# tigert1998/ray-tracing-cuda

Hardware: AMD Instinct MI355X
Metric: Mrays/s (higher is better)
Workload: dtype f32

## Files before the change

### include/rtmi.h

```cpp
#ifndef RTMI_H_
#define RTMI_H_

#include <stddef.h>
#include <stdint.h>

#ifdef __cplusplus
extern "C" {
#endif

#define RTMI_VERSION 3
#define RTMI_TILE 8
#define RTMI_STATE_WORDS 6

typedef enum rtmi_status {
  RTMI_OK = 0,
  RTMI_ERR_INVALID = -1,
  RTMI_ERR_NO_DEVICE = -2,
  RTMI_ERR_HIP = -3,
  RTMI_ERR_CAPACITY = -4,
  RTMI_ERR_DEPTH = -5,
  RTMI_ERR_INTERNAL = -6
} rtmi_status;

#define RTMI_MAX_DEPTH 64
// ... 94 lines not shown

int rtmi_post_process(float *d_image, int64_t n_pixels, int spp, void *stream);
int rtmi_get_workload(int rank, int world_size, int spp);

int rtmi_selftest_arithmetic(unsigned long long mismatches[8]);

typedef struct rtmi_render_opts {
  int32_t size;
  int32_t schedule;
  int32_t blocks_per_cu;
  int32_t threads_per_block;
  int32_t sparse_stride;
  int32_t exclusive;
  int32_t outlier_x10;
  int32_t probe_spp;
  int32_t head_pct[3];
  int32_t plan;
  int32_t wave_priority;
  int32_t lane_stride;
  int32_t promote_after;
  int32_t cost_probe;
  int32_t first_pass;
  int32_t fast_path;
  void *d_scratch;
  size_t scratch_bytes;
} rtmi_render_opts;
size_t rtmi_render_scratch_bytes(const rtmi_frame *f);
int rtmi_render_launch_shape(const rtmi_scene *s, const rtmi_frame *f, const rtmi_render_opts *opts, int32_t out[4]);
int rtmi_render_mode(const rtmi_scene *s, const rtmi_frame *f, const rtmi_render_opts *opts, int32_t out[8]);
#define RTMI_MODE_FIELDS 9
int rtmi_render_mode_ex(const rtmi_scene *s, const rtmi_frame *f, const rtmi_render_opts *opts, int32_t *out, int n);
#define RTMI_FAST_PATH_FACTS 14
int rtmi_fast_path_kernel(const int32_t facts[RTMI_FAST_PATH_FACTS]);
int rtmi_render_ex(const rtmi_scene *s, const rtmi_frame *f, const rtmi_render_opts *opts, void *d_states,
                   float *d_tiles, uint32_t *d_ray_counts, void *stream);

enum {
  RTMI_HIT_NONE = 0,
  RTMI_HIT_SPHERE = 1,
  RTMI_HIT_TRIANGLE = 2,
  RTMI_HIT_PARALLELOGRAM = 3,
  RTMI_HIT_PARALLELEPIPED = 4,
  RTMI_HIT_MESH = 5,
  RTMI_HIT_SKY = 6
};
typedef struct rtmi_hit {
  float t;
  float u, v;
  float normal[3];
  int32_t material;
  int32_t kind;
  int32_t entry;
  int32_t element;
  int32_t reserved[2];
} rtmi_hit;

int rtmi_intersect(const rtmi_scene *s, int64_t n, const float *d_origins, const float *d_dirs,
                   const float *d_t_max, rtmi_hit *d_hits, unsigned long long *d_abandoned, void *stream);

int rtmi_occluded(const rtmi_scene *s, int64_t n, const float *d_origins, const float *d_dirs, const float *d_t_max,
                  uint8_t *d_occluded, unsigned long long *d_counts, void *stream);

#define RTMI_TRACE_WORK_WORDS 256
int rtmi_trace(const rtmi_scene *s, int64_t n, const float *d_origins, const float *d_dirs, int max_depth,
               void *d_states, float *d_radiance, uint32_t *d_ray_counts, unsigned long long *d_work, void *stream);
int rtmi_rng_init_n(uint64_t seed, uint64_t first, int64_t n, void *d_states, void *stream);
// ... 177 lines not shown
```

### ray-tracing-cuda_amd/csrc/capi.hip

```cpp
#include <hip/hip_runtime.h>
#include <dlfcn.h>
#include <rccl/rccl.h>
#include <string.h>

#include <algorithm>
#include <cmath>
#include <cstdlib>
#include <mutex>
#include <string>
#include <type_traits>
#include <unordered_map>

#include "../../include/rtmi.h"
#include "kernels.h"
#include "scene.h"
#include "xorwow.h"

using namespace rtmi;

static thread_local std::string g_err;
static int fail(int code, const std::string &msg) {
  g_err = msg;
  return code;
}
// ... 351 lines not shown
int rtmi_camera_set(rtmi_scene *s, const float f[21], int is_defocus, double lens_radius) {
  if (!s || !f) return fail(RTMI_ERR_INVALID, "null argument");
  CameraDev &c = S(s)->cam;
  c.position = v3(f), c.llc = v3(f + 3), c.horizontal = v3(f + 6), c.vertical = v3(f + 9);
  c.u = v3(f + 12), c.v = v3(f + 15);
  S(s)->cam_w = v3(f + 18);
  c.defocus = is_defocus ? 1 : 0;
  c.lens_radius = (float)lens_radius;
  S(s)->has_camera = true;
  S(s)->committed = false;
  return RTMI_OK;
}
int rtmi_camera_update(rtmi_scene *s, const float f[21], int is_defocus, double lens_radius) {
  if (!s || !f) return fail(RTMI_ERR_INVALID, "null argument");
  if (!all_finite(f, 21)) return fail(RTMI_ERR_INVALID, "non-finite camera float");
  Scene *sc = S(s);
  const bool committed = sc->committed;
  if (int rc = rtmi_camera_set(s, f, is_defocus, lens_radius)) return rc;
  if (committed) {
    sc->dev.cam = sc->cam;
    sc->features = sc->cam.defocus ? sc->features | F_DEFOCUS : sc->features & ~(uint32_t)F_DEFOCUS;
    sc->committed = true;
  }
  return RTMI_OK;
}
int rtmi_camera_get(const rtmi_scene *s, float out[21]) {
  if (!s || !out || !S(s)->has_camera) return fail(RTMI_ERR_INVALID, "scene has no camera");
  const CameraDev &c = S(s)->cam;
  const V3 vs[7] = {c.position, c.llc, c.horizontal, c.vertical, c.u, c.v, S(s)->cam_w};
  for (int i = 0; i < 7; i++) out[i * 3] = vs[i].x, out[i * 3 + 1] = vs[i].y, out[i * 3 + 2] = vs[i].z;
  return RTMI_OK;
}

int rtmi_scene_commit(rtmi_scene *sp) {
  if (!sp) return fail(RTMI_ERR_INVALID, "null scene");
  Scene *s = S(sp);
  if (s->list_counts.size() != 1) return fail(RTMI_ERR_INVALID, "a nested list is still open (rtmi_list_end missing)");
  static_assert(RTMI_MAX_MATERIALS == kMaxMats, "rtmi.h and scene_dev.h disagree on the material limit");
  if (s->mats.size() > (size_t)RTMI_MAX_MATERIALS)
    return fail(RTMI_ERR_CAPACITY, "more than RTMI_MAX_MATERIALS (2^24) materials: a triangle's material field has 24 bits");
  if (rtmi_device_count() <= 0) return fail(RTMI_ERR_NO_DEVICE, "no HIP device: librtmi has no CPU fallback");
  free_device(s);
  std::string err = s->flatten();
  if (!err.empty()) return fail(RTMI_ERR_INVALID, err);
  HIP_TRY(hipGetDevice(&s->device));
  s->tex_recs.clear();
  for (const HostTex &t : s->texs) {
    if (!t.image) continue;
    void *d = nullptr;
    size_t pitch = 0;
    HIP_TRY(hipMallocPitch(&d, &pitch, (size_t)t.w * 4, (size_t)t.h));
    s->dev_allocs.push_back(d);
    HIP_TRY(hipMemcpy2D(d, pitch, t.rgba.data(), (size_t)t.w * 4, (size_t)t.w * 4, (size_t)t.h,
                        hipMemcpyHostToDevice));
    TexRec r{};
    r.rgba = reinterpret_cast<const uint8_t *>(d);
    r.height = t.h, r.width = t.w, r.pitch = (int64_t)pitch;
    s->tex_recs.push_back(r);
  }
  SceneDev d{};
  int rc;
  if ((rc = upload(s, s->runs, &d.runs))) return rc;
  if ((rc = upload(s, s->spheres, &d.spheres))) return rc;
  if ((rc = upload(s, s->tris, &d.tris))) return rc;
  {
    static_assert(sizeof(PairSlab) == sizeof(PairBox) && std::is_trivially_copyable<PairSlab>::value, "PairSlab records travel as PairBox");
// ... 12 lines not shown
  if ((rc = upload(s, s->nodes, &d.nodes))) return rc;
  if ((rc = upload(s, s->qnodes, &d.qnodes))) return rc;
  if ((rc = upload(s, s->leaf_paths, &d.leaf_paths))) return rc;
  if ((rc = upload(s, s->tops, &d.tops))) return rc;
  if ((rc = upload(s, s->faces, &d.faces))) return rc;
  if ((rc = upload(s, s->face_uv, &d.face_uv))) return rc;
#ifdef RTMI_CHECK_MARGINS
  if ((rc = upload(s, s->face_of_orig, &d.face_of_orig))) return rc;
#endif
  if ((rc = upload(s, s->mat_recs, &d.mats))) return rc;
  if ((rc = upload(s, s->tex_recs, &d.texs))) return rc;
  d.n_runs = (int)s->runs.size() - 4;
  d.n_pairs = (int)s->pair_pts.size();
  d.list_mag = s->list_mag;
  d.n_mats = (int)s->mat_recs.size();
  d.n_nodes = (int)s->nodes.size();
  d.n_leaf_paths = (int)s->leaf_paths.size();
  d.sub_reserve = s->sub_depth > 0 ? 3 * s->sub_depth + 3 + kMeshFaceSlack : 0;
  d.det_safe = 1;
  for (const HotTri &t : s->tris) {
    const double a = std::sqrt((double)t.e1[0] * t.e1[0] + (double)t.e1[1] * t.e1[1] + (double)t.e1[2] * t.e1[2]);
    const double b = std::sqrt((double)t.e2[0] * t.e2[0] + (double)t.e2[1] * t.e2[1] + (double)t.e2[2] * t.e2[2]);
    if (!(a * b <= 0x1p120)) d.det_safe = 0;
  }
  d.unsigned_colours = 1;
  for (const MatRec &m : s->mat_recs) {
    const float c[3] = {m.r, m.g, m.b};
    for (float x : c) {
      uint32_t bits;
      memcpy(&bits, &x, sizeof(bits));
      if (bits >> 31) d.unsigned_colours = 0;
    }
  }
  d.cam = s->cam;
  s->dev = d;
  QueryDev q{};
  if ((rc = upload(s, s->q_sphere_entry, &q.sphere_entry))) return rc;
  if ((rc = upload(s, s->q_pair_entry, &q.pair_entry))) return rc;
  if ((rc = upload(s, s->q_bvh_entry, &q.bvh_entry))) return rc;
  if ((rc = upload(s, s->q_face_input, &q.face_input))) return rc;
  q.sky_entry = s->q_sky_entry;
  s->qdev = q;
  {
    std::vector<uint32_t> light_mats;
    std::vector<LightRec> recs;
    std::vector<float> cdf;
    build_light_table(*s, &s->lights, &light_mats);
    light_records(s->lights, &recs, &cdf);
    LightDev l{};
    if ((rc = upload(s, recs, &l.recs))) return rc;
    if ((rc = upload(s, cdf, &l.cdf))) return rc;
    if ((rc = upload(s, light_mats, &l.light_mats))) return rc;
    l.n_lights = (int32_t)s->lights.size(), l.n_mats = (int32_t)s->mat_recs.size();
    std::vector<int32_t> hit_light;
    build_hit_light_map(s->lights, &hit_light, &l.n_entries);
    if ((rc = upload(s, hit_light, &l.hit_light))) return rc;
    s->ldev = l;
  }
  void *c = nullptr;
  HIP_TRY(hipMalloc(&c, RTMI_COUNTER_WORDS * sizeof(unsigned long long) + 2 * render_params_bytes()));
  s->dev_allocs.push_back(c);
  HIP_TRY(hipMemset(c, 0, RTMI_COUNTER_WORDS * sizeof(unsigned long long)));
  s->d_counters = reinterpret_cast<unsigned long long *>(c);
  HIP_TRY(hipDeviceSynchronize());
  s->committed = true;
  return RTMI_OK;
// ... 35 lines not shown
}

int64_t rtmi_debug_list_records(const rtmi_scene *sp, int64_t cap_pairs, uint32_t *tri_pts, uint32_t *hot_tris, float *corners) {
  if (!sp) return fail(RTMI_ERR_INVALID, "null scene");
  Scene tmp;
  if (int rc = flattened(sp, &tmp)) return rc;
  const int64_t n = (int64_t)tmp.pair_pts.size();
  for (int64_t i = 0; i < n && i < cap_pairs; i++) {
    if (tri_pts) memcpy(tri_pts + 24 * i, &tmp.tri_pts[2 * i], 2 * sizeof(TriPts));
    if (hot_tris) memcpy(hot_tris + 32 * i, &tmp.tris[2 * i], 2 * sizeof(HotTri));
    if (corners) memcpy(corners + 12 * i, tmp.pair_pts[i].p0, 12 * sizeof(float));
  }
  return n;
}

int64_t rtmi_debug_pair_slabs(const rtmi_scene *sp, int64_t cap, uint32_t *slabs, uint32_t *boxes, float *list_mag) {
  if (!sp) return fail(RTMI_ERR_INVALID, "null scene");
  Scene tmp;
  if (int rc = flattened(sp, &tmp)) return rc;
  const int64_t n = (int64_t)tmp.pair_slabs.size();
  for (int64_t i = 0; i < n && i < cap; i++) {
    if (slabs) memcpy(slabs + 8 * i, &tmp.pair_slabs[i], sizeof(PairSlab));
    if (boxes) memcpy(boxes + 8 * i, &tmp.pair_boxes[i], sizeof(PairBox));
  }
  if (list_mag) *list_mag = tmp.list_mag;
  return n;
}

int rtmi_debug_slab_reach(const rtmi_scene *sp) {
  if (!sp) return fail(RTMI_ERR_INVALID, "null scene");
  Scene tmp;
  if (int rc = flattened(sp, &tmp)) return rc;
  return slab_reach_covers(tmp.list_mag, tmp.cam) ? 1 : 0;
}

int64_t rtmi_debug_render_lds_bytes(const rtmi_scene *sp, int max_depth, int threads) {
  if (!sp || max_depth < 0 || threads < 64 || threads % 64) return fail(RTMI_ERR_INVALID, "bad arguments");
  Scene tmp;
  if (int rc = flattened(sp, &tmp)) return rc;
  SceneDev d{};
  d.n_pairs = (int)tmp.pair_pts.size(), d.n_mats = (int)tmp.mat_recs.size(), d.n_nodes = (int)tmp.nodes.size();
  d.n_leaf_paths = (int)tmp.leaf_paths.size(), d.n_sph_groups = (int)tmp.sph_groups.size();
  FrameDev fr{};
  fr.max_depth = max_depth;
  return (int64_t)render_lds_bytes(pick_variant(tmp.features), d, fr, threads);
}

int64_t rtmi_frame_work_items(const rtmi_frame *f) {
  FrameDev d;
  if (!make_frame(f, &d)) return fail(RTMI_ERR_INVALID, frame_why("bad frame"));
  return d.items;
}
int64_t rtmi_frame_pixel_of(const rtmi_frame *f, int64_t q) {
  FrameDev d;
  if (!make_frame(f, &d) || q < 0 || q >= d.items) return -1;
  return frame_pixel_of(d, d.rank, q);
}
int rtmi_frame_pixel_map(const rtmi_frame *f, int64_t *out) {
  FrameDev d;
  if (!make_frame(f, &d) || !out) return fail(RTMI_ERR_INVALID, frame_why("bad frame"));
  for (int64_t q = 0; q < d.items; q++) out[q] = frame_pixel_of(d, d.rank, q);
  return RTMI_OK;
}
size_t rtmi_states_bytes(const rtmi_frame *f) {
  FrameDev d;
  if (!make_frame(f, &d)) return 0;
// ... 245 lines not shown
  p->scratch = p->scheduled || p->prio;
  p->first = p->finish = d;
  p->first.k_end = probe_spp;
  if (p->resume) p->finish.k_begin = probe_spp;
  else p->first.spp = probe_spp;
  p->first_fast = fast_mode(ls.fast, ls.lane_stride, p->first_prio, false, false, false);
  p->finish_fast = fast_mode(ls.fast, ls.lane_stride, p->prio, p->chains, p->resume, p->scheduled);
  return RTMI_OK;
}

int rtmi_render_launch_shape(const rtmi_scene *sp, const rtmi_frame *f, const rtmi_render_opts *opts, int32_t out[4]) {
  if (!sp || !out) return fail(RTMI_ERR_INVALID, "null argument");
  RenderPlan p;
  int rc;
  if ((rc = render_prologue(sp, f, opts, &p)) || (rc = plan_render(&p))) return rc;
  out[0] = p.ls.blocks, out[1] = p.ls.threads, out[2] = p.ls.per_cu, out[3] = p.ls.n_cu;
  return RTMI_OK;
}

int rtmi_render_mode(const rtmi_scene *sp, const rtmi_frame *f, const rtmi_render_opts *opts, int32_t out[8]) {
  return rtmi_render_mode_ex(sp, f, opts, out, 8);
}
int rtmi_render_mode_ex(const rtmi_scene *sp, const rtmi_frame *f, const rtmi_render_opts *opts, int32_t *dst, int n) {
  if (!sp || !dst || n < 0) return fail(RTMI_ERR_INVALID, "null argument");
  RenderPlan p;
  int rc;
  if ((rc = render_prologue(sp, f, opts, &p)) || (rc = plan_render(&p))) return rc;
  const int32_t out[RTMI_MODE_FIELDS] = {p.scheduled, p.scheduled ? p.probe_spp : 0, p.resume, p.chains, p.prio ? p.tune.prio_every : 0,
                                         p.ls.lane_stride, p.waves, p.d.local_tiles, p.finish_fast != 0u};
  for (int i = 0; i < n && i < RTMI_MODE_FIELDS; i++) dst[i] = out[i];
  return RTMI_OK;
}

struct Scratch {
  uint32_t *states, *rays, *cost, *order, *meta, *head, *work, *qcost, *qsorted, *qmap, *qmax, *fut, *claims, *prio_tab;
  int32_t *next, *first;
};
static Scratch scratch_regions(void *base, const ScratchLayout &l) {
  const auto at = [base](size_t off) { return reinterpret_cast<uint32_t *>(static_cast<char *>(base) + off); };
  const auto ints = [&at](size_t off) { return reinterpret_cast<int32_t *>(at(off)); };
  return Scratch{at(l.states), at(l.rays), at(l.cost), at(l.order), at(l.meta), at(l.head), at(l.work), at(l.qcost), at(l.qsorted),
                 at(l.qmap), at(l.qmax), at(l.fut), at(l.claims), at(l.prio_tab), ints(l.next), ints(l.first)};
}

struct SchedStep {
  int tiles;
  bool pixel_head;
  uint32_t sparse_cap;
  int waves, outlier_x10;
  const int *head_pct;
  int simds, rounds;
  int spp, probe_spp;
};
static int schedule_step(const Scratch &r, uint32_t *rays, const uint32_t *work, const SchedStep &k, SchedPlan *plan,
                         hipStream_t st) {
  uint32_t *head = k.pixel_head ? r.head : nullptr;
  HIP_TRY(launch_tile_order(rays, k.tiles, r.cost, r.meta, r.order, head, k.sparse_cap, k.waves, k.outlier_x10, k.head_pct, st));
  HIP_TRY(launch_quarter_order(r.order, work, rays, k.tiles, r.qcost, r.qsorted, r.qmax, r.qmap, st));
  plan->tile_order = r.qmap;
  plan->sparse_items = r.meta + 1;
  plan->head_list = head;
  plan->probe_marks = head ? rays : nullptr;
  plan->probe_spp = k.probe_spp;
  plan->tile_cost = r.cost;
  if ((int64_t)k.simds * k.rounds > 0) {
    HIP_TRY(launch_chain_plan(r.order, r.cost, k.tiles, k.simds, k.rounds, k.spp, k.probe_spp, r.first, r.next, r.fut, st));
// ... 903 lines not shown
```

### ray-tracing-cuda_amd/csrc/kernels.h

```cpp
#pragma once
#include <hip/hip_runtime.h>
#include <stdint.h>

#include <vector>

#include "../../include/rtmi.h"
#include "scene_dev.h"

#define RTMI_KERNEL_MAX_DEPTH 64

namespace rtmi {

#include "path_list.h"

int64_t frame_pixel_of(const FrameDev &fr, int rank, int64_t q);

hipError_t launch_rng_init(uint64_t seed, const FrameDev &fr, const uint32_t *d_jump, uint32_t *d_states,
                           hipStream_t stream, int64_t first = -1);

uint32_t pick_variant(uint32_t features);
int render_occupancy(uint32_t variant, const SceneDev &sc, const FrameDev &fr, int threads, bool fast_path = false);
struct RenderTuning {
  int schedule;
  int blocks_per_cu;
  int threads;
  int sparse_stride;
  int exclusive;
  int outlier_x10;
  int head_pct[3];
  int probe_spp;
  int promote;
  int first_pass;
  int cost_probe;
  int lane_stride;
  int plan;
  int prio_every;
  int fast_path;
  int head_classes;
  int first_prio;
  int fetch_batch, fetch_batch_first;
};

enum : uint32_t {
  PIN_NIBBLE_IDS = 1u << 0,
  PIN_LDS_TABLES = 1u << 1,
  PIN_UNSIGNED = 1u << 2,
  PIN_DET_SAFE = 1u << 3,
  PIN_POW2_FRAME = 1u << 4,
  PIN_EVERY_LANE = 1u << 5,
  PIN_PRIORITIES = 1u << 6,
  PIN_CHAINS = 1u << 7,
  PIN_QUEUE = 1u << 8,
};
constexpr uint32_t kFastCommon = PIN_NIBBLE_IDS | PIN_LDS_TABLES | PIN_UNSIGNED | PIN_DET_SAFE | PIN_POW2_FRAME |
                                 PIN_EVERY_LANE | PIN_PRIORITIES;
constexpr uint32_t kFastChains = kFastCommon | PIN_CHAINS;
constexpr uint32_t kFastQueue = kFastCommon | PIN_QUEUE;
constexpr bool defers_unit(uint32_t m) { return (m & kFastCommon) == kFastCommon; }
constexpr bool culls_by_slab(uint32_t m) { return (m & kFastCommon) == kFastCommon; }
constexpr bool folds_by_min(uint32_t m) { return (m & kFastCommon) == kFastCommon; }
#ifndef RTMI_TRIM
#define RTMI_TRIM 7
#endif
constexpr bool trims_votes(uint32_t m) { return (RTMI_TRIM & 1) && (m & kFastCommon) == kFastCommon; }
constexpr bool trims_mul24(uint32_t m) { return (RTMI_TRIM & 2) && (m & kFastCommon) == kFastCommon; }
constexpr bool trims_fold_rgb(uint32_t m) { return (RTMI_TRIM & 4) && (m & kFastCommon) == kFastCommon; }
constexpr int kFoldRgbOff = 512;
constexpr int kFoldRgbBytes = 256;
constexpr int kOrderedTasksWord = 16;
struct FastPathFacts {
  int enabled;
  uint32_t variant;
  int n_mats;
  int mats_in_lds;
  int pairs_in_lds;
  int unsigned_colours;
  int det_safe;
  int width, height;
  int lane_stride;
  int priorities;
  int chains;
  int resumed;
  int tile_cost;
};
uint32_t fast_path_mode(const FastPathFacts &f);
FastPathFacts fast_path_facts(uint32_t variant, const SceneDev &sc, const FrameDev &fr, int threads, int enabled);
bool slab_reach_covers(float list_mag, const CameraDev &cam);
size_t render_lds_bytes(uint32_t variant, const SceneDev &sc, const FrameDev &fr, int threads);
struct SchedPlan {
  const uint32_t *tile_order = nullptr;
  uint32_t *visit_counts = nullptr;
  const uint32_t *sparse_items = nullptr;
  const uint32_t *head_list = nullptr;
  const uint32_t *probe_marks = nullptr;
  int probe_spp = 2;
  uint32_t *prio_tab = nullptr;
  const uint32_t *tile_cost = nullptr;
  const int32_t *chain_next = nullptr;
  const uint32_t *chain_fut = nullptr;
// ... 122 lines not shown
```

### ray-tracing-cuda_amd/csrc/render.hip

```cpp
#include <hip/hip_runtime.h>
#include <stdint.h>

#include "kernels.h"

#include <cfloat>
#include <cmath>
#include <cstdlib>
#include <iterator>
#include <type_traits>
#include "scene_dev.h"
#include "vec.h"
#include "xorwow.h"

namespace rtmi {

#include "frame_math.h"
#include "trace_helpers.h"
#include "path_shared.h"
#include "mesh_search.h"
#include "closest_hit.h"
#include "render_body.h"
#include "launch_cfg.h"

size_t render_params_bytes() { return (sizeof(RenderParams) + 255) & ~(size_t)255; }
// ... 85 lines not shown
bool slab_reach_covers(float list_mag, const CameraDev &cam) {
  const float reach = kOriginReach * list_mag;
  const bool cam_in_reach = fabsf(cam.position.x) <= reach && fabsf(cam.position.y) <= reach && fabsf(cam.position.z) <= reach;
  const bool k_finite = (double)(kOriginReach + 1.0f) * (double)list_mag * 1e30 < (double)FLT_MAX;
  return cam_in_reach && k_finite;
}
FastPathFacts fast_path_facts(uint32_t variant, const SceneDev &sc, const FrameDev &fr, int threads, int enabled) {
  size_t lds = 0;
  const LaunchCfg lc = make_cfg(variant, sc, fr, threads, &lds);
  FastPathFacts f{};
  f.enabled = enabled, f.variant = variant, f.n_mats = sc.n_mats, f.mats_in_lds = lc.lds_mats > 0 && lc.wide_ids == 2;
  f.pairs_in_lds = lc.pairs_off >= 0 && lc.nrm_off >= 0 && lc.list_off >= 0 && slab_reach_covers(sc.list_mag, sc.cam);
  f.unsigned_colours = sc.unsigned_colours, f.det_safe = sc.det_safe, f.width = fr.width, f.height = fr.height;
  return f;
}

size_t render_lds_bytes(uint32_t variant, const SceneDev &sc, const FrameDev &fr, int threads) {
  size_t lds = 0;
  (void)make_cfg(variant, sc, fr, threads, &lds);
  return lds;
}

int render_occupancy(uint32_t variant, const SceneDev &sc, const FrameDev &fr, int threads, bool fast_path) {
  return with_listed<kVariants>(variant, 0, [&](auto v) {
    constexpr uint32_t F = decltype(v)::value;
    size_t lds = 0;
    (void)make_cfg(F, sc, fr, threads, &lds);
    if (threads > RTMI_MAX_THREADS(F)) return 0;
    int nb = 0;
    (void)kernel_occupancy<render_kernel<F>>(threads, lds, &nb);
    if constexpr (F == (uint32_t)F_TRIS) {
      if (fast_path) {
        int nc = 0, nq = 0;
        (void)kernel_occupancy<render_kernel<F, kFastChains>>(threads, lds, &nc);
        (void)kernel_occupancy<render_kernel<F, kFastQueue>>(threads, lds, &nq);
        nb = nb < nc ? nb : nc, nb = nb < nq ? nb : nq;
      }
    }
    return nb;
  });
}

int image_order_batch(int samples, int cap) {
  const int per_atomic = samples < 32 ? 256 / (samples > 0 ? samples : 1) : 64 / samples;
  return per_atomic < 1 ? 1 : per_atomic > cap ? cap : per_atomic;
}

hipError_t launch_render(uint32_t variant, const SceneDev &sc, const FrameDev &fr, uint32_t *d_states, float *d_out,
                         uint32_t *d_ray_counts, unsigned long long *d_counters, const SchedPlan &plan, bool probe,
                         uint32_t fast, int blocks, int threads, const RenderTuning &tune, void *d_params, hipStream_t stream) {
  return with_listed<kVariants>(variant, hipErrorInvalidValue, [&](auto v) {
    constexpr uint32_t F = decltype(v)::value;
    size_t lds = 0;
    LaunchCfg lc = make_cfg(F, sc, fr, threads, &lds);
    lc.tile_order = plan.tile_order;
    lc.visit_counts = plan.visit_counts;
    lc.sparse_items = plan.sparse_items;
    lc.head_list = plan.head_list;
    lc.probe_marks = plan.probe_marks;
    lc.sparse_stride = tune.sparse_stride;
    lc.exclusive = tune.exclusive;
    lc.probe_spp = plan.probe_spp;
    lc.promote = tune.promote;
    lc.lane_stride = tune.lane_stride > 0 ? tune.lane_stride : 1;
    lc.prio_tab = plan.prio_tab;
    lc.tile_cost = plan.tile_cost;
    lc.rate_scale = 1.f / (64.f * (float)(plan.probe_spp > 0 ? plan.probe_spp : 1));
    lc.chain_next = (F & F_BVH) || lc.prio_tab == nullptr ? nullptr : plan.chain_next;
    lc.chain_fut = plan.chain_fut, lc.chain_first = plan.chain_first, lc.claims = plan.claims;
    lc.plan_simds = plan.plan_simds, lc.plan_rounds = plan.plan_rounds;
    lc.prio_every = tune.prio_every > 0 ? tune.prio_every : 16;
    {
      const int samples = fr.k_end - fr.k_begin > 0 ? fr.k_end - fr.k_begin : 1;
      const int by_length = 4096 / samples < 1 ? 1 : 4096 / samples;
      lc.fetch_batch = probe && samples <= 4 ? tune.fetch_batch_first : plan.tile_order != nullptr ? std::min(by_length, tune.fetch_batch) : image_order_batch(samples, 16);
    }
    RenderParams rp;
    rp.sc = sc, rp.fr = fr, rp.lc = lc;
    rp.states = d_states, rp.out = d_out, rp.ray_counts = d_ray_counts, rp.counters = d_counters;
    RenderParams *dp = reinterpret_cast<RenderParams *>(d_params);
    const LaunchAt at{blocks, threads, lds, stream};
    if constexpr (F == (uint32_t)F_TRIS) {
      const bool chains = fast == kFastChains && !probe && lc.chain_next && lc.tile_cost && fr.k_begin > 0 && d_ray_counts;
      const bool queue = fast == kFastQueue && !lc.chain_next;
      if (fast != 0u && (!lc.prio_tab || lc.lane_stride != 1 || !(chains || queue))) return hipErrorInvalidValue;
      if (fast != 0u && lc.stack_off != kFoldRgbOff + kFoldRgbBytes) return hipErrorInvalidValue;
      static_assert(culls_by_slab(kFastChains) && culls_by_slab(kFastQueue) && !culls_by_slab(0u), "which kernels read the slab table");
      if (chains || queue) rp.sc.pair_boxes = pair_slabs_of(sc.pair_boxes, sc.n_pairs);
      if (chains) return launch_block<render_kernel<F, kFastChains>>(at, rp, dp);
      if (queue && !probe) return launch_block<render_kernel<F, kFastQueue>>(at, rp, dp);
      if (queue) return launch_block<probe_kernel<F, kFastQueue>>(at, rp, dp);
    }
    if (fast != 0u) return hipErrorInvalidValue;
    if (probe) return launch_block<probe_kernel<F>>(at, rp, dp);
    return launch_block<render_kernel<F>>(at, rp, dp);
  });
}

}
```

### ray-tracing-cuda_amd/csrc/render_body.h

```cpp
#pragma once

struct QueryHit;
template <uint32_t F>
__device__ __forceinline__ QueryHit resolve_hit(const SceneDev &sc, const QueryDev &qd, const Hit &h, V3 o, V3 d);

struct LaunchCfg {
  int32_t lds_mats;
  int32_t wide_ids;
  int32_t stack_off;
  int32_t nodes_off;
  int32_t lds_nodes;
  int32_t mesh_off;
  int32_t exclusive;
  int32_t pairs_off;
  int32_t list_off;
  int32_t paths_off;
  int32_t lds_paths;
  int32_t threads;
  int32_t nrm_off;
  int32_t probe_spp;
  int32_t promote;
  int32_t cand_off;
  const uint32_t *tile_order;
  uint32_t *visit_counts;
// ... 196 lines not shown
    int *dst = reinterpret_cast<int *>(smem + lc.paths_off);
    for (int w = threadIdx.x; w < lc.lds_paths; w += blockDim.x) dst[w] = sc.leaf_paths[w];
  }
  __syncthreads();

  const int64_t n_items = fr.items;
  const bool w_pow2 = (fr.width & (fr.width - 1)) == 0, h_pow2 = (fr.height & (fr.height - 1)) == 0;
  const double inv_w = 1.0 / (double)fr.width, inv_h = 1.0 / (double)fr.height;
  const bool f32_jitter = (M & PIN_POW2_FRAME) || (w_pow2 && h_pow2 && fr.width <= (1 << 20) && fr.height <= (1 << 20));
  int32_t q32 = -1;
  uint32_t work_px = 0;
  uint32_t ray_acc = 0;
  uint32_t pij = 0;
  int k = 0;
  bool has_px = false, done = false, active = false;
  bool heavy = false;
  V3 color = splat(0.f);
  V3 moment = splat(0.f);
  int k_end_px = 0;
  auto k_end = [&]() -> int {
    if constexpr (BUDGET) return k_end_px;
    else return fr.k_end;
  };
  auto feature_add3 = [&](float *buf, V3 v) {
    float *w = buf + (int64_t)q32 * 3;
    w[0] = __fadd_rn(w[0], v.x), w[1] = __fadd_rn(w[1], v.y), w[2] = __fadd_rn(w[2], v.z);
  };
  uint32_t rays = 0;
  Rng rng = {0, 0, 0, 0, 0, 0};
  V3 o = splat(0.f), d = splat(0.f);
  int depth = 0;
  constexpr bool DEFER = defers_unit(M);
  constexpr int kOwesBit = (int)0x80000000u;
  const bool tex32 = (F & F_TEX) && (!QUEUE || tex_layers);
  auto tex_layer_offset = [&](int level) -> uint32_t {
    return (uint32_t)lc.stack_off + (((uint32_t)level * n_threads + threadIdx.x) << 2);
  };

  unsigned long long sparse_limit = 0ull;
  if ((F & F_BVH) && lc.sparse_items) sparse_limit = *lc.sparse_items;
  const bool classes = (F & F_BVH) && lc.head_list != nullptr && sparse_limit != 0ull;
  uint32_t end64 = 0u, end32 = 0u;
  if (classes) end64 = lc.sparse_items[1], end32 = lc.sparse_items[2];
  uint32_t thr64 = 0xffffffffu, thr32 = 0xffffffffu, thr16 = 0xffffffffu;
  if (classes && lc.exclusive && lc.promote) thr64 = lc.sparse_items[23], thr32 = lc.sparse_items[24], thr16 = lc.sparse_items[25];
  const bool promote = thr16 != 0xffffffffu;
  int cls = 1;
  bool head_open = classes;
  auto take_item = [&](int64_t item) -> bool {
    q32 = (int32_t)item;
    const int64_t q = item;
    if constexpr (RAYS) {
      V3 ro, rd;
      if constexpr (STEP) {
        ro = mk(step->origins[q * 3 + 0], step->origins[q * 3 + 1], step->origins[q * 3 + 2]);
        rd = mk(step->dirs[q * 3 + 0], step->dirs[q * 3 + 1], step->dirs[q * 3 + 2]);
      } else {
        ro = mk(ray_o[q * 3 + 0], ray_o[q * 3 + 1], ray_o[q * 3 + 2]);
        rd = mk(ray_d[q * 3 + 0], ray_d[q * 3 + 1], ray_d[q * 3 + 2]);
      }
      bool live = finite3(ro) && finite3(rd) && (rd.x != 0.f || rd.y != 0.f || rd.z != 0.f);
      V3 nd = splat(0.f);
      if (live) nd = unit3_rn(rd);
      live = live && finite3(nd) && (nd.x != 0.f || nd.y != 0.f || nd.z != 0.f);
      if (!live) {
        if constexpr (!STEP) {
// ... 272 lines not shown
        float r1 = rng_01(rng);
        float r2 = rng_01(rng);
        float xf, yf;
        if (f32_jitter) {
          xf = (r1 + (float)(pij & 0xffffu)) * (float)inv_w;
          yf = (r2 + (float)(fr.height - (int)(pij >> 16))) * (float)inv_h;
        } else {
          double x = (double)r1 + (double)(int)(pij & 0xffffu);
          double y = (double)r2 + (double)(fr.height - (int)(pij >> 16));
          x = w_pow2 ? x * inv_w : x / (double)fr.width;
          y = h_pow2 ? y * inv_h : y / (double)fr.height;
          x = 2 * x - 1;
          y = 2 * y - 1;
          x = (x + 1) / 2;
          y = (y + 1) / 2;
          xf = (float)x, yf = (float)y;
        }
        V3 target = sc.cam.llc + xf * sc.cam.horizontal + yf * sc.cam.vertical;
        V3 origin = sc.cam.position;
        if (F & F_DEFOCUS) {
          if (sc.cam.defocus) {
            float ox = rng_range(0.f, sc.cam.lens_radius, rng);
            float oy = rng_range(0.f, sc.cam.lens_radius, rng);
            origin = sc.cam.position + sc.cam.u * ox + sc.cam.v * oy;
          }
        }
        o = origin;
        d = DEFER ? target - origin : unit3_rn_twice(target - origin);
        k++;
        if ((F & F_BVH) && promote && cls == 1 && k >= lc.promote) {
          const unsigned long long have = (unsigned long long)rays * (unsigned)lc.probe_spp, per = (unsigned long long)k;
          if (have >= thr16 * per) cls = have >= thr64 * per ? 64 : have >= thr32 * per ? 32 : 16;
        }
        depth = DEFER ? kOwesBit : 0;
        active = true;
      }
    }
    if constexpr (DEFER) {
      if (depth < 0) {
        d = unit3_rn_twice<VOTE>(d);
        depth &= ~kOwesBit;
      }
    }
    if (!__any(active)) {
      if (!(F & F_BVH) || __all(done)) break;
      continue;
    }

#if defined(RTMI_STATS) && RTMI_STATS == 9
    if ((wave_queries + 1u) % 600u == 0u && (wave_queries + 1u) / 600u <= 9u && (threadIdx.x & 63u) == 0u)
      g_wave_stats[((blockIdx.x * blockDim.x + threadIdx.x) >> 6) & 16383u][(wave_queries + 1u) / 600u] =
          ((stat_real() - t_begin) & 0xffffffffffull) | ((unsigned long long)(st.node_steps + st.face_steps) << 40);
#endif
    RTMI_STAT(wave_queries++; const unsigned long long tq1 = stat_now(); st.cyc[0] += tq1 - tq0;
              const unsigned long long in0 = st.cyc[2] + st.cyc[3];)
    Hit h = {};
    const bool all_lanes_in = (F & F_BVH) || ((F & F_TRIS) && ((M & PIN_LDS_TABLES) || (ll != nullptr && sc.n_pairs >= kCullMinPairs))) ||
                              ((F & F_SGROUP) && cands != nullptr);
    if (all_lanes_in)
      h = closest_hit<F, false, M>(sc, s_nodes, lc.lds_nodes, s_paths, lc.lds_paths, s_tris, ll, cands, wl, counters + (QUEUE ? 0 : 2), o, d, active,
                         (F & F_BVH) && lc.visit_counts != nullptr
#ifdef RTMI_STATS
                         , st
#endif
      );
    RTMI_STAT(const unsigned long long tq2 = stat_now(); st.cyc[1] += (tq2 - tq1) - (st.cyc[2] + st.cyc[3] - in0);)
#ifdef RTMI_CHECK_MARGINS
    if (!QUEUE && all_lanes_in && (check_tick++ % RTMI_CHECK_EVERY) == 0u) {
      const Hit h2 = closest_hit<F>(sc, s_nodes, 0, s_paths, 0, nullptr, nullptr, nullptr, nullptr, nullptr, o, d, active, false
#ifdef RTMI_STATS
                                    , st
#endif
      );
      const bool differs = active && (h2.ok != h.ok || (h.ok && (__float_as_uint(h2.t) != __float_as_uint(h.t) || h2.win != h.win ||
                                                                 ((F & F_BVH) && h2.aux != h.aux))));
      const unsigned long long na = __builtin_amdgcn_ballot_w64(active), nd = __builtin_amdgcn_ballot_w64(differs);
      if ((threadIdx.x & 63u) == 0u) {
        atomicAdd(&counters[33], (unsigned long long)__popcll(na));
        if (nd) atomicAdd(&counters[34], (unsigned long long)__popcll(nd));
      }
    }
#endif
    if (active) {
      if (!all_lanes_in)
        h = closest_hit<F, false, M & ~(uint32_t)PIN_LDS_TABLES>(sc, s_nodes, 0, s_paths, 0, s_tris, nullptr, nullptr, nullptr, nullptr, o, d, true, false
#ifdef RTMI_STATS
                           , st
#endif
        );
      rays++;
      if ((F & F_BVH) && lc.visit_counts != nullptr) work_px += (uint32_t)h.work;

      V3 result = splat(0.f);
      bool ended = true;
      V3 step_att = splat(0.f), step_o = o, step_d = splat(0.f);
      if (h.ok && depth < fr.max_depth) {
        const uint32_t kind = h.win >> 29;
        const uint32_t index = h.win & ID_INDEX_MASK;
        V3 p = o + h.t * d;
        if (kind == RUN_SKY) {
          V3 dir = unit3_rn<VOTE>(p);
          float tg = (float)(0.5 * ((double)dir.y + 1.0));
          float w0 = 1.0f - tg;
          result = mk(w0 * 1.0f + tg * 0.5f, w0 * 1.0f + tg * 0.7f, w0 * 1.0f + tg * 1.0f);
          if constexpr (FEATURES) {
            if (depth == 0 && feat->albedo) feature_add3(feat->albedo, result);
          }
        } else {
          V3 nrm = splat(0.f);
          int mat = 0;
          float tu = 0.f, tv = 0.f;
          if ((F & F_TRIS) && kind == RUN_TRIS) {
            V3 n;
            int flags;
            if ((M & PIN_LDS_TABLES) || s_tris != nullptr) {
              const float4 tn = s_nrm[index];
              n = mk(tn.x, tn.y, tn.z);
              mat = __float_as_int(tn.w) & 0xffffff, flags = __float_as_int(tn.w) >> 24;
            } else {
              const HotTri &tr = sc.tris[index];
              n = mk(tr.n[0], tr.n[1], tr.n[2]);
              mat = tr.mat, flags = tr.flags;
            }
            nrm = dot3(d, n) < 0.f ? n : -n;
            if (F & F_TEX) {
              if (flags & TRI_PGRAM) {
                float w = (float)((1.0 - (double)h.u) - (double)h.v);
                if (!(flags & TRI_SECOND)) {
                  tu = (0.f * w + 1.f * h.u) + 0.f * h.v;
// ... 223 lines not shown
          }
        }
        for (; !FOLD4 && i >= 0; i--) {
          V3 a;
          if (tex32) {
            const uint32_t lw = *reinterpret_cast<const uint32_t *>(smem + tex_layer_offset(i));
            if (lw >> 31) {
              a = texel_rgb(lw);
            } else if (mats_in_lds) {
              a = lds_rgb((int)lw);
            } else {
              a = mk(sc.mats[lw].r, sc.mats[lw].g, sc.mats[lw].b);
            }
          } else {
            const int mi = nibble_ids     ? (int)((smem[ids_offset(i >> 1)] >> ((i & 1) * 4)) & 15u)
                           : lc.wide_ids ? (int)*reinterpret_cast<const uint16_t *>(smem + ids_offset(i))
                                         : (int)smem[ids_offset(i)];
            if (mats_in_lds) {
              a = lds_rgb(mi);
            } else {
              a = mk(sc.mats[mi].r, sc.mats[mi].g, sc.mats[mi].b);
            }
          }
          if (sc.unsigned_colours) {
            result = mk(a.x * result.x, a.y * result.y, a.z * result.z);
          } else {
            result = mk(0.f + a.x * result.x, 0.f + a.y * result.y, 0.f + a.z * result.z);
          }
        }
        color = color + result;
        if constexpr (BUDGET)
          moment = mk(__fadd_rn(moment.x, __fmul_rn(result.x, result.x)), __fadd_rn(moment.y, __fmul_rn(result.y, result.y)),
                      __fadd_rn(moment.z, __fmul_rn(result.z, result.z)));
        active = false;
      }
    }
    RTMI_STAT(st.cyc[4] += stat_now() - tq2;)
  }

  if (RTMI_PRIO) wave_priority_leave(lc.prio_tab);
#undef RTMI_CHAINS
#undef RTMI_PRIO
  {
    unsigned long long ray_total = ray_acc;
    for (int off = 32; off > 0; off >>= 1) ray_total += __shfl_down(ray_total, off);
    if ((threadIdx.x & 63) == 0 && ray_total) atomicAdd(&counters[1], ray_total);
  }
#ifdef RTMI_STATS
  if (!QUEUE && (threadIdx.x & 63) == 0) {
    const unsigned v[13] = {wave_queries, st.searches, st.node_steps, st.face_steps, st.nodes_popped, st.blocks_popped,
                            st.insert_rounds, st.steps_hist[0], st.steps_hist[1], st.steps_hist[2], st.steps_hist[3],
                            st.steps_hist[4], st.steps_hist[5]};
    for (int i = 0; i < 13; i++) atomicAdd(&counters[4 + i], (unsigned long long)v[i]);
    for (int i = 0; i < 9; i++) atomicAdd(&counters[17 + i], st.cyc[i]);
    const unsigned long long life = stat_real() - t_begin;
    atomicAdd(&counters[26], life);
    atomicMax(&counters[27], life);
    atomicAdd(&counters[28], 1ull);
    atomicAdd(&counters[29], st.calib);
    atomicAdd(&counters[30], st.cull_bits);
    atomicAdd(&counters[31], st.cull_iters);
    atomicAdd(&counters[32], st.cull_rays);
    for (int i = 0; i < 3; i++)
      atomicAdd(&counters[37 + i], (unsigned long long)st.nnow_hist[2 * i] | ((unsigned long long)st.nnow_hist[2 * i + 1] << 32));
    for (int i = 0; i < 4 && !(F & F_BVH); i++)
      atomicAdd(&counters[12 + i], (unsigned long long)st.trip_hist[2 * i] | ((unsigned long long)st.trip_hist[2 * i + 1] << 32));
    const unsigned wid = (blockIdx.x * blockDim.x + threadIdx.x) >> 6;
// ... 20 lines not shown
```

### ray-tracing-cuda_amd/csrc/scene_dev.h

```cpp
#pragma once
#include <stdint.h>

#include "vec.h"
#include "margins.h"

namespace rtmi {

enum RunKind : int32_t { RUN_SKY = 0, RUN_SPHERE = 1, RUN_TRIS = 2, RUN_BVH = 4 };

struct Run {
  int32_t kind, first, count, pad;
};

struct SphereRec {
  float cx, cy, cz;
  int32_t mat;
  double radius;
  double r2;
};

struct SphGroup {
  float mn[3], mx[3];
  int32_t first, count;
};
struct SphMember {
  float cx, cy, cz;
  float r2f;
  int32_t orig;
  int32_t pad;
  double r2;
};
constexpr int kSphGroupSize = 16;
constexpr int kSphGroupMin = 32;
// ... 121 lines not shown
  uint32_t code;
  int32_t leaf;
};

struct CameraDev {
  V3 position, llc, horizontal, vertical, u, v;
  float lens_radius;
  int32_t defocus;
};

constexpr int kPrioRows = 1 << 14;
constexpr size_t kPrioTabBytes = (size_t)kPrioRows * 16 * sizeof(uint32_t);

constexpr int kLdsMats = 512;
constexpr int kLdsNodes = 512;

struct SceneDev {
  const Run *runs;
  const SphereRec *spheres;
  const HotTri *tris;
  const PairBox *pair_boxes;
  const SphGroup *sph_groups;
  const SphMember *sph_members;
  float sph_mag;
  int32_t n_sph_groups;
  const TriPts *tri_pts;
  const TriNrm *tri_nrm;
  const BvhRec *bvhs;
  const BvhNode *nodes;
  const QNode4 *qnodes;
  const BvhNode *tops;
  const int32_t *leaf_paths;
  int32_t n_leaf_paths;
  const FaceRec *faces;
  const float *face_uv;
#ifdef RTMI_CHECK_MARGINS
  const int32_t *face_of_orig;
#endif
  const MatRec *mats;
  const TexRec *texs;
  int32_t n_runs, n_mats, n_nodes;
  int32_t n_pairs;
  float list_mag;
  int32_t sub_reserve;
  int32_t det_safe;
  int32_t unsigned_colours;
  CameraDev cam;
};

enum : int32_t { QHIT_NONE = 0, QHIT_SPHERE = 1, QHIT_TRIANGLE = 2, QHIT_PARALLELOGRAM = 3, QHIT_PARALLELEPIPED = 4,
                 QHIT_MESH = 5, QHIT_SKY = 6 };
struct QueryDev {
  const int32_t *sphere_entry;
  const int32_t *pair_entry;
  const int32_t *bvh_entry;
  const int32_t *face_input;
  int32_t sky_entry;
};

enum : uint32_t {
  F_SPHERE = 1u,
  F_TRIS = 2u,
  F_SGROUP = 4u,
  F_BVH = 8u,
  F_TEX = 16u,
  F_DEFOCUS = 32u,
  F_ALL = 63u
};

struct FrameDev {
  int32_t height, width, spp, max_depth, post;
  int32_t k_begin, k_end;
  int32_t rank, world;
  int32_t tiles_x, tiles_y, n_tiles;
  int32_t local_tiles;
  int64_t items;
};

struct FeatureBufs {
  float *albedo = nullptr;
  float *normal = nullptr;
// ... 6 lines not shown
```

### ray-tracing-cuda_amd/rtmi/_abi.py

```python
import ctypes as C
import os

import numpy as np

_PKG_DIR = os.path.dirname(os.path.abspath(__file__))
_ROOT = os.path.dirname(_PKG_DIR)
LIB_PATH = os.environ.get("RTMI_LIB_PATH") or os.path.join(_ROOT, "lib", "librtmi.so")

TILE = 8
STATE_WORDS = 6
MAX_DEPTH = 64
TRACE_WORK_WORDS = 256
BUDGET_WORK_WORDS = TRACE_WORK_WORDS
PATH_COMPACT_ITEMS = 1024
MODE_FIELDS = 9
FAST_PATH_FACTS = 14
MAX_MATERIALS = 1 << 24
SHADOW_DEFAULT = "list"

RTMI_HIT_NONE = 0
RTMI_HIT_SPHERE = 1
RTMI_HIT_TRIANGLE = 2
RTMI_HIT_PARALLELOGRAM = 3
RTMI_HIT_PARALLELEPIPED = 4
# ... 132 lines not shown
    ("rtmi_add_parallelepiped", C.c_int, [C.c_void_p, _fp, C.c_int]),
    ("rtmi_add_parallelepiped_lengths", C.c_int, [C.c_void_p, _fp, C.c_int, TRANSFORM_FN, C.c_void_p]),
    ("rtmi_add_parallelepiped_faces", C.c_int, [C.c_void_p, _fp, C.c_int]),
    ("rtmi_add_sky", C.c_int, [C.c_void_p]),
    ("rtmi_list_begin", C.c_int, [C.c_void_p]),
    ("rtmi_list_end", C.c_int, [C.c_void_p]),
    ("rtmi_add_bvh", C.c_int, [C.c_void_p, _fp, _fp, C.c_int, C.c_int, C.c_int]),
    ("rtmi_camera_pinhole", C.c_int, [C.c_void_p, _fp, _fp, _fp, C.c_double, C.c_double]),
    ("rtmi_camera_defocus", C.c_int, [C.c_void_p, _fp, _fp, _fp, C.c_double, C.c_double, C.c_double, C.c_double]),
    ("rtmi_camera_raw", C.c_int, [C.c_void_p, _fp, _fp, _fp, _fp]),
    ("rtmi_camera_get", C.c_int, [C.c_void_p, _fp]),
    ("rtmi_camera_set", C.c_int, [C.c_void_p, _fp, C.c_int, C.c_double]),
    ("rtmi_scene_commit", C.c_int, [C.c_void_p]),
    ("rtmi_scene_stats", C.c_int, [C.c_void_p, C.POINTER(C.c_int64)]),
    ("rtmi_scene_bytes_per_ray", C.c_int64, [C.c_void_p]),
    ("rtmi_scene_sliver_faces", C.c_int64, [C.c_void_p]),
    ("rtmi_frame_work_items", C.c_int64, [_frp]),
    ("rtmi_frame_pixel_of", C.c_int64, [_frp, C.c_int64]),
    ("rtmi_frame_pixel_map", C.c_int, [_frp, C.POINTER(C.c_int64)]),
    ("rtmi_states_bytes", C.c_size_t, [_frp]),
    ("rtmi_tiles_bytes", C.c_size_t, [_frp]),
    ("rtmi_rng_init", C.c_int, [C.c_uint64, _frp, C.c_void_p, C.c_void_p]),
    ("rtmi_rng_host_state", C.c_int, [C.c_uint64, C.c_uint64, _u32p]),
    ("rtmi_rng_host_random_float", C.c_float, [C.c_float, C.c_float, _u32p]),
    ("rtmi_rng_set_state", C.c_int, [_frp, C.c_void_p, C.c_int64, _u32p, C.c_void_p]),
    ("rtmi_rng_get_state", C.c_int, [_frp, C.c_void_p, C.c_int64, _u32p, C.c_void_p]),
    ("rtmi_render", C.c_int, [C.c_void_p, _frp, C.c_void_p, C.c_void_p, C.c_void_p, C.c_void_p]),
    ("rtmi_render_ex", C.c_int, [C.c_void_p, _frp, C.POINTER(RenderOpts), C.c_void_p, C.c_void_p, C.c_void_p, C.c_void_p]),
    ("rtmi_render_scratch_bytes", C.c_size_t, [_frp]),
    ("rtmi_render_launch_shape", C.c_int, [C.c_void_p, _frp, C.POINTER(RenderOpts), C.POINTER(C.c_int32)]),
    ("rtmi_render_mode", C.c_int, [C.c_void_p, _frp, C.POINTER(RenderOpts), C.POINTER(C.c_int32)]),
    ("rtmi_render_mode_ex", C.c_int, [C.c_void_p, _frp, C.POINTER(RenderOpts), C.POINTER(C.c_int32), C.c_int]),
    ("rtmi_fast_path_kernel", C.c_int, [C.POINTER(C.c_int32)]),
    ("rtmi_render_status", C.c_int, [C.c_void_p, C.c_void_p, C.POINTER(C.c_uint64), C.c_void_p]),
    ("rtmi_last_ray_total", C.c_int, [C.c_void_p, C.POINTER(C.c_uint64), C.c_void_p]),
    ("rtmi_debug_counters", C.c_int, [C.c_void_p, C.POINTER(C.c_ulonglong), C.c_void_p]),
    ("rtmi_debug_counters_ex", C.c_int, [C.c_void_p, C.c_void_p, C.POINTER(C.c_ulonglong), C.c_void_p]),
    ("rtmi_debug_scratch_regions", C.c_int, [_frp, C.POINTER(C.c_int64), C.c_int]),
    ("rtmi_debug_schedule", C.c_int, [_frp, C.c_void_p, C.c_size_t, C.c_void_p, C.c_void_p, C.c_int, C.c_uint32, C.c_int, C.c_int,
                                      C.POINTER(C.c_int32), C.c_int, C.c_int, C.c_int, C.c_int, C.c_void_p]),
    ("rtmi_gather", C.c_int, [C.c_void_p, _frp, C.c_void_p, C.c_void_p, C.c_int, C.c_void_p]),
    ("rtmi_reduce_sum", C.c_int, [C.c_void_p, _frp, C.c_void_p, C.c_int, C.c_void_p]),
    ("rtmi_untile", C.c_int, [_frp, C.c_void_p, C.c_void_p, C.c_void_p]),
    ("rtmi_untile_u32", C.c_int, [_frp, C.c_void_p, C.c_void_p, C.c_void_p]),
    ("rtmi_post_process", C.c_int, [C.c_void_p, C.c_int64, C.c_int, C.c_void_p]),
    ("rtmi_get_workload", C.c_int, [C.c_int, C.c_int, C.c_int]),
    ("rtmi_selftest_arithmetic", C.c_int, [C.POINTER(C.c_ulonglong)]),
    ("rtmi_set_launch", C.c_int, [C.c_int, C.c_int]),
    ("rtmi_set_schedule", C.c_int, [C.c_int]),
    ("rtmi_intersect", C.c_int, [C.c_void_p, C.c_int64, C.c_void_p, C.c_void_p, C.c_void_p, C.c_void_p, C.c_void_p,
                                 C.c_void_p]),
    ("rtmi_occluded", C.c_int, [C.c_void_p, C.c_int64, C.c_void_p, C.c_void_p, C.c_void_p, C.c_void_p, C.c_void_p,
                                C.c_void_p]),
    ("rtmi_trace", C.c_int, [C.c_void_p, C.c_int64, C.c_void_p, C.c_void_p, C.c_int, C.c_void_p, C.c_void_p, C.c_void_p,
                             C.c_void_p, C.c_void_p]),
    ("rtmi_rng_init_n", C.c_int, [C.c_uint64, C.c_uint64, C.c_int64, C.c_void_p, C.c_void_p]),
    ("rtmi_render_budget", C.c_int, [C.c_void_p, _frp, C.c_void_p, C.c_void_p, C.c_void_p, C.c_void_p, C.c_void_p,
                                     C.c_void_p, C.c_void_p, C.c_void_p]),
    ("rtmi_budget_plan", C.c_int, [_frp, C.POINTER(AdaptiveOpts), C.c_void_p, C.c_void_p, C.c_void_p, C.c_void_p,
                                   C.c_void_p, C.c_void_p]),
    ("rtmi_resolve", C.c_int, [_frp, C.c_void_p, C.c_void_p, C.c_int, C.c_void_p, C.c_void_p]),
    ("rtmi_render_features", C.c_int, [C.c_void_p, _frp, C.c_void_p, C.c_void_p, C.c_void_p, C.c_void_p, C.c_void_p,
                                       C.c_void_p, C.POINTER(Features), C.c_void_p, C.c_void_p]),
    ("rtmi_resolve_features", C.c_int, [_frp, C.POINTER(Features), C.c_void_p, C.POINTER(Features), C.c_void_p]),
    ("rtmi_resolve_variance", C.c_int, [_frp, C.c_void_p, C.c_void_p, C.c_void_p, C.c_void_p, C.c_void_p]),
    ("rtmi_denoise_scratch_bytes", C.c_size_t, [C.c_int, C.c_int]),
# ... 95 lines not shown
```

Baseline: 38510.

## Add specialised diffuse-only fast render kernel with in-place sample restarts

Detects scenes whose materials are all untextured Lambertian or light and pins a specialised variant of the fast list render kernels. The variant uses a trimmed shading path (sky, light or Lambertian scatter only), normalises the direction eagerly instead of through the deferred owes-bit, and, when a path ends, immediately starts the lane's next sample from the camera rather than going idle. The aim is to cut per-bounce branching and register pressure and to keep lanes busy. It adds more kernel instantiations and a specialised code path whose RNG consumption must match the general one.

```diff
diff --git a/include/rtmi.h b/include/rtmi.h
--- a/include/rtmi.h
+++ b/include/rtmi.h
@@ -150,6 +150,7 @@
 int rtmi_render_mode_ex(const rtmi_scene *s, const rtmi_frame *f, const rtmi_render_opts *opts, int32_t *out, int n);
 #define RTMI_FAST_PATH_FACTS 14
 int rtmi_fast_path_kernel(const int32_t facts[RTMI_FAST_PATH_FACTS]);
+int rtmi_render_pins(const rtmi_scene *s, const rtmi_frame *f, const rtmi_render_opts *opts, uint32_t out[2]);
 int rtmi_render_ex(const rtmi_scene *s, const rtmi_frame *f, const rtmi_render_opts *opts, void *d_states,
                    float *d_tiles, uint32_t *d_ray_counts, void *stream);
 
diff --git a/ray-tracing-cuda_amd/csrc/capi.hip b/ray-tracing-cuda_amd/csrc/capi.hip
--- a/ray-tracing-cuda_amd/csrc/capi.hip
+++ b/ray-tracing-cuda_amd/csrc/capi.hip
@@ -407,6 +407,12 @@
   return RTMI_OK;
 }
 
+static int diffuse_only(const std::vector<MatRec> &mats) {
+  for (const MatRec &m : mats)
+    if ((m.kind != MAT_LAMBERTIAN && m.kind != MAT_LIGHT) || m.tex >= 0) return 0;
+  return 1;
+}
+
 int rtmi_scene_commit(rtmi_scene *sp) {
   if (!sp) return fail(RTMI_ERR_INVALID, "null scene");
   Scene *s = S(sp);
@@ -485,6 +491,7 @@
       if (bits >> 31) d.unsigned_colours = 0;
     }
   }
+  d.diffuse_only = diffuse_only(s->mat_recs);
   d.cam = s->cam;
   s->dev = d;
   QueryDev q{};
@@ -586,6 +593,13 @@
   Scene tmp;
   if (int rc = flattened(sp, &tmp)) return rc;
   return slab_reach_covers(tmp.list_mag, tmp.cam) ? 1 : 0;
+}
+
+int rtmi_debug_diffuse_only(const rtmi_scene *sp) {
+  if (!sp) return fail(RTMI_ERR_INVALID, "null scene");
+  Scene tmp;
+  if (int rc = flattened(sp, &tmp)) return rc;
+  return diffuse_only(tmp.mat_recs);
 }
 
 int64_t rtmi_debug_render_lds_bytes(const rtmi_scene *sp, int max_depth, int threads) {
@@ -897,6 +911,16 @@
   return RTMI_OK;
 }
 
+int rtmi_render_pins(const rtmi_scene *sp, const rtmi_frame *f, const rtmi_render_opts *opts, uint32_t out[2]) {
+  if (!sp || !out) return fail(RTMI_ERR_INVALID, "null argument");
+  RenderPlan p;
+  int rc;
+  if ((rc = render_prologue(sp, f, opts, &p)) || (rc = plan_render(&p))) return rc;
+  out[0] = p.scheduled ? render_pins(p.first_fast, p.s->dev) : 0u;
+  out[1] = render_pins(p.finish_fast, p.s->dev);
+  return RTMI_OK;
+}
+
 struct Scratch {
   uint32_t *states, *rays, *cost, *order, *meta, *head, *work, *qcost, *qsorted, *qmap, *qmax, *fut, *claims, *prio_tab;
   int32_t *next, *first;
diff --git a/ray-tracing-cuda_amd/csrc/kernels.h b/ray-tracing-cuda_amd/csrc/kernels.h
--- a/ray-tracing-cuda_amd/csrc/kernels.h
+++ b/ray-tracing-cuda_amd/csrc/kernels.h
@@ -51,6 +51,7 @@
   PIN_PRIORITIES = 1u << 6,
   PIN_CHAINS = 1u << 7,
   PIN_QUEUE = 1u << 8,
+  PIN_DIFFUSE = 1u << 9,
 };
 constexpr uint32_t kFastCommon = PIN_NIBBLE_IDS | PIN_LDS_TABLES | PIN_UNSIGNED | PIN_DET_SAFE | PIN_POW2_FRAME |
                                  PIN_EVERY_LANE | PIN_PRIORITIES;
@@ -65,6 +66,12 @@
 constexpr bool trims_votes(uint32_t m) { return (RTMI_TRIM & 1) && (m & kFastCommon) == kFastCommon; }
 constexpr bool trims_mul24(uint32_t m) { return (RTMI_TRIM & 2) && (m & kFastCommon) == kFastCommon; }
 constexpr bool trims_fold_rgb(uint32_t m) { return (RTMI_TRIM & 4) && (m & kFastCommon) == kFastCommon; }
+#ifndef RTMI_DIFFUSE
+#define RTMI_DIFFUSE 5
+#endif
+constexpr bool diffuse_scatter(uint32_t m) { return (RTMI_DIFFUSE & 1) && (m & PIN_DIFFUSE) && (m & kFastCommon) == kFastCommon; }
+constexpr bool diffuse_restarts(uint32_t m) { return (RTMI_DIFFUSE & 4) && diffuse_scatter(m); }
+inline uint32_t render_pins(uint32_t fast, const SceneDev &sc) { return fast != 0u && sc.diffuse_only ? fast | PIN_DIFFUSE : fast; }
 constexpr int kFoldRgbOff = 512;
 constexpr int kFoldRgbBytes = 256;
 constexpr int kOrderedTasksWord = 16;
diff --git a/ray-tracing-cuda_amd/csrc/render.hip b/ray-tracing-cuda_amd/csrc/render.hip
--- a/ray-tracing-cuda_amd/csrc/render.hip
+++ b/ray-tracing-cuda_amd/csrc/render.hip
@@ -141,8 +141,13 @@
     if constexpr (F == (uint32_t)F_TRIS) {
       if (fast_path) {
         int nc = 0, nq = 0;
-        (void)kernel_occupancy<render_kernel<F, kFastChains>>(threads, lds, &nc);
-        (void)kernel_occupancy<render_kernel<F, kFastQueue>>(threads, lds, &nq);
+        if (sc.diffuse_only) {
+          (void)kernel_occupancy<render_kernel<F, kFastChains | PIN_DIFFUSE>>(threads, lds, &nc);
+          (void)kernel_occupancy<render_kernel<F, kFastQueue | PIN_DIFFUSE>>(threads, lds, &nq);
+        } else {
+          (void)kernel_occupancy<render_kernel<F, kFastChains>>(threads, lds, &nc);
+          (void)kernel_occupancy<render_kernel<F, kFastQueue>>(threads, lds, &nq);
+        }
         nb = nb < nc ? nb : nc, nb = nb < nq ? nb : nq;
       }
     }
@@ -196,6 +201,11 @@
       if (fast != 0u && lc.stack_off != kFoldRgbOff + kFoldRgbBytes) return hipErrorInvalidValue;
       static_assert(culls_by_slab(kFastChains) && culls_by_slab(kFastQueue) && !culls_by_slab(0u), "which kernels read the slab table");
       if (chains || queue) rp.sc.pair_boxes = pair_slabs_of(sc.pair_boxes, sc.n_pairs);
+      if (render_pins(fast, sc) & PIN_DIFFUSE) {
+        if (chains) return launch_block<render_kernel<F, kFastChains | PIN_DIFFUSE>>(at, rp, dp);
+        if (queue && !probe) return launch_block<render_kernel<F, kFastQueue | PIN_DIFFUSE>>(at, rp, dp);
+        if (queue) return launch_block<probe_kernel<F, kFastQueue | PIN_DIFFUSE>>(at, rp, dp);
+      }
       if (chains) return launch_block<render_kernel<F, kFastChains>>(at, rp, dp);
       if (queue && !probe) return launch_block<render_kernel<F, kFastQueue>>(at, rp, dp);
       if (queue) return launch_block<probe_kernel<F, kFastQueue>>(at, rp, dp);
diff --git a/ray-tracing-cuda_amd/csrc/render_body.h b/ray-tracing-cuda_amd/csrc/render_body.h
--- a/ray-tracing-cuda_amd/csrc/render_body.h
+++ b/ray-tracing-cuda_amd/csrc/render_body.h
@@ -252,6 +252,8 @@
   int depth = 0;
   constexpr bool DEFER = defers_unit(M);
   constexpr int kOwesBit = (int)0x80000000u;
+  constexpr bool DIFF = diffuse_scatter(M), DIFF_RESTARTS = diffuse_restarts(M);
+  static_assert(!DIFF || (DEFER && FOLD4 && (M & PIN_POW2_FRAME)), "the diffuse kernels are fast list kernels");
   const bool tex32 = (F & F_TEX) && (!QUEUE || tex_layers);
   auto tex_layer_offset = [&](int level) -> uint32_t {
     return (uint32_t)lc.stack_off + (((uint32_t)level * n_threads + threadIdx.x) << 2);
@@ -590,11 +592,13 @@
           const unsigned long long have = (unsigned long long)rays * (unsigned)lc.probe_spp, per = (unsigned long long)k;
           if (have >= thr16 * per) cls = have >= thr64 * per ? 64 : have >= thr32 * per ? 32 : 16;
         }
-        depth = DEFER ? kOwesBit : 0;
+        depth = DEFER && !DIFF ? kOwesBit : 0;
         active = true;
       }
     }
-    if constexpr (DEFER) {
+    if constexpr (DIFF) {
+      if (active) d = unit3_rn_twice<VOTE>(d);
+    } else if constexpr (DEFER) {
       if (depth < 0) {
         d = unit3_rn_twice<VOTE>(d);
         depth &= ~kOwesBit;
@@ -652,7 +656,69 @@
       V3 result = splat(0.f);
       bool ended = true;
       V3 step_att = splat(0.f), step_o = o, step_d = splat(0.f);
-      if (h.ok && depth < fr.max_depth) {
+      [[maybe_unused]] bool restart = false;
+      if constexpr (DIFF) {
+        bool scatters = false;
+        V3 p = o, nrm = splat(0.f);
+        uint32_t mat = 0u;
+        if (h.ok && depth < fr.max_depth) {
+          const uint32_t index = h.win & ID_INDEX_MASK;
+          p = o + h.t * d;
+          if ((h.win >> 29) == RUN_SKY) {
+            V3 dir = unit3_rn<VOTE>(p);
+            float tg = (float)(0.5 * ((double)dir.y + 1.0));
+            float w0 = 1.0f - tg;
+            result = mk(w0 * 1.0f + tg * 0.5f, w0 * 1.0f + tg * 0.7f, w0 * 1.0f + tg * 1.0f);
+          } else {
+            const float4 tn = s_nrm[index];
+            const V3 n = mk(tn.x, tn.y, tn.z);
+            mat = (uint32_t)__float_as_int(tn.w) & 0xffffffu;
+            nrm = dot3(d, n) < 0.f ? n : -n;
+            const float4 m0 = load_lds<float4>(s_mats + mat);
+            if (__float_as_int(m0.w) == MAT_LIGHT) {
+              result = mk(m0.x, m0.y, m0.z);
+            } else {
+              scatters = !(dot3(d, nrm) >= 0.f);
+            }
+          }
+        }
+        if constexpr (DIFF_RESTARTS) restart = !scatters && k < k_end();
+        if (scatters || restart) {
+          [[maybe_unused]] uint32_t ux = 0u, uy = 0u;
+          float sum = 0.f;
+          V3 b = splat(0.f);
+          if constexpr (DIFF_RESTARTS) {
+            ux = rng_next(rng), uy = rng_next(rng);
+            if (scatters) {
+              float x = rng_pm1_of(ux), y = rng_pm1_of(uy), z = rng_pm1(rng);
+              sum = x * x + y * y + z * z;
+              while (sum > BALL_S_MAX) {
+                x = rng_pm1(rng), y = rng_pm1(rng), z = rng_pm1(rng);
+                sum = x * x + y * y + z * z;
+              }
+              b = mk(x, y, z);
+            }
+          } else {
+            b = ball_sample(rng, sum);
+          }
+          if (!DIFF_RESTARTS || scatters) {
+            const V3 s = sampler_on_sphere<VOTE>(b, sum);
+            const uint32_t at = ids_offset(depth >> 1);
+            const uint32_t old = smem[at];
+            smem[at] = (uint8_t)((depth & 1) ? ((old & 0x0fu) | (mat << 4)) : ((old & 0xf0u) | mat));
+            depth++;
+            o = p;
+            d = s + nrm;
+            ended = false;
+          } else {
+            const float xf = (rng_01_of(ux) + (float)(pij & 0xffffu)) * (float)inv_w;
+            const float yf = (rng_01_of(uy) + (float)(fr.height - (int)(pij >> 16))) * (float)inv_h;
+            const V3 target = sc.cam.llc + xf * sc.cam.horizontal + yf * sc.cam.vertical;
+            o = sc.cam.position;
+            d = target - sc.cam.position;
+          }
+        }
+      } else if (h.ok && depth < fr.max_depth) {
         const uint32_t kind = h.win >> 29;
         const uint32_t index = h.win & ID_INDEX_MASK;
         V3 p = o + h.t * d;
@@ -942,7 +1008,8 @@
         if constexpr (BUDGET)
           moment = mk(__fadd_rn(moment.x, __fmul_rn(result.x, result.x)), __fadd_rn(moment.y, __fmul_rn(result.y, result.y)),
                       __fadd_rn(moment.z, __fmul_rn(result.z, result.z)));
-        active = false;
+        if (DIFF_RESTARTS && restart) k++, depth = 0;
+        else active = false;
       }
     }
     RTMI_STAT(st.cyc[4] += stat_now() - tq2;)
diff --git a/ray-tracing-cuda_amd/csrc/scene_dev.h b/ray-tracing-cuda_amd/csrc/scene_dev.h
--- a/ray-tracing-cuda_amd/csrc/scene_dev.h
+++ b/ray-tracing-cuda_amd/csrc/scene_dev.h
@@ -1,4 +1,5 @@
 #pragma once
+#include <stddef.h>
 #include <stdint.h>
 
 #include "vec.h"
@@ -186,6 +187,7 @@
   const BvhNode *tops;
   const int32_t *leaf_paths;
   int32_t n_leaf_paths;
+  int32_t diffuse_only;
   const FaceRec *faces;
   const float *face_uv;
 #ifdef RTMI_CHECK_MARGINS
@@ -201,6 +203,9 @@
   int32_t unsigned_colours;
   CameraDev cam;
 };
+static_assert(offsetof(SceneDev, diffuse_only) + sizeof(int32_t) == offsetof(SceneDev, faces) &&
+              offsetof(SceneDev, diffuse_only) == offsetof(SceneDev, n_leaf_paths) + sizeof(int32_t),
+              "diffuse_only fills the padding between n_leaf_paths and faces");
 
 enum : int32_t { QHIT_NONE = 0, QHIT_SPHERE = 1, QHIT_TRIANGLE = 2, QHIT_PARALLELOGRAM = 3, QHIT_PARALLELEPIPED = 4,
                  QHIT_MESH = 5, QHIT_SKY = 6 };
diff --git a/ray-tracing-cuda_amd/rtmi/_abi.py b/ray-tracing-cuda_amd/rtmi/_abi.py
--- a/ray-tracing-cuda_amd/rtmi/_abi.py
+++ b/ray-tracing-cuda_amd/rtmi/_abi.py
@@ -188,6 +188,7 @@
     ("rtmi_render_mode", C.c_int, [C.c_void_p, _frp, C.POINTER(RenderOpts), C.POINTER(C.c_int32)]),
     ("rtmi_render_mode_ex", C.c_int, [C.c_void_p, _frp, C.POINTER(RenderOpts), C.POINTER(C.c_int32), C.c_int]),
     ("rtmi_fast_path_kernel", C.c_int, [C.POINTER(C.c_int32)]),
+    ("rtmi_render_pins", C.c_int, [C.c_void_p, _frp, C.POINTER(RenderOpts), _u32p]),
     ("rtmi_render_status", C.c_int, [C.c_void_p, C.c_void_p, C.POINTER(C.c_uint64), C.c_void_p]),
     ("rtmi_last_ray_total", C.c_int, [C.c_void_p, C.POINTER(C.c_uint64), C.c_void_p]),
     ("rtmi_debug_counters", C.c_int, [C.c_void_p, C.POINTER(C.c_ulonglong), C.c_void_p]),
```

After: 39130, median of 6. +1.6%, better.
